# R-Sweke/DeepQ-Decoding

Hardware: AMD Instinct MI355X
Metric: env steps/sec + DQN updates/sec, d=5 depolarising, batch 4096, 1/2/4/8 GPU (higher is better)
Workload: dtype f32 (operands as 2 f16 pieces = 22 significant bits, 2 or 3 f16 MFMAs per product, f32 accumulate); 1 GPU; c3: d=5 DP p_phys=p_meas=0.011 depth=5, 4096 lattices/GPU, mode=loop; policy=eps-greedy over legal moves, eps=0.1, live Q-network, minibatch_per_gpu=4096, updates_per_vector_step=1, observations=patch words (d*d u32 per lattice), replay_ring_slots=257, network=conv 64x3s2-32x2-32x2, dense 512 (dropout .2), dueling, n_params=193283, grad_allreduce=none (1 GPU)

## Files before the change

deepq-decoding_amd/csrc/fused.hip:

```cpp
#include "qnet.h"
#include <type_traits>
#include <utility>

DQ_STAMP_READER(dq_dbg_read_fwd)

#ifndef CONV_PIN
#define CONV_PIN 1
#endif
#ifndef DENSE_PIN
#define DENSE_PIN 1
#endif
#ifndef CONV_APIPE
#define CONV_APIPE 1
#endif
#ifndef DENSE_XPIPE
#define DENSE_XPIPE 1
#endif
#ifndef CONV_SWZ
#define CONV_SWZ 0
#endif
#define A1_PS (CONV_SWZ ? 64 : 72)
#ifndef CONV1_PIPE
#define CONV1_PIPE 0
#endif
// ... 961 lines not shown
    const int NTQ = (A + 15) >> 4;
    float b3[KG3][4];
    f32x4 bias1[4];
#pragma unroll
    for (int ct = 0; ct < 4; ++ct)
        bias1[ct] = *reinterpret_cast<const f32x4u*>(J.params + a.b_off[0] + 64 * wave + 32 * (ct >> 1) + 8 * kq + 4 * (ct & 1));
    const int nt3 = NTQ > 0 ? NTQ : 1, parts = DENSE_WAVES / nt3, ct3 = wave % nt3, part = wave / nt3;
    const bool act3 = a.N3 > 0 && part < parts;
    const int col3 = 16 * ct3 + j;
    float bias3 = 0.f;
    auto load_b3 = [&]() {
        const float* w3q = reinterpret_cast<const float*>(J.packed + a.pk_w3q);
        bias3 = w3q[16 * KG3 * PW + col3];
#pragma unroll
        for (int g = 0; g < KG3; ++g)
#pragma unroll
            for (int s = 0; s < 4; ++s) b3[g][s] = w3q[(16 * g + 4 * kq + s) * PW + col3];
    };
    if (act3 && !LEAN) load_b3();
    const int rcol = tid & 63;
    float bias2r[(PW + 63) / 64];
#pragma unroll
    for (int cc = 0; cc < (PW + 63) / 64; ++cc) bias2r[cc] = J.params[a.b_off[1] + min(rcol + 64 * cc, a.N2 - 1)];
    __syncthreads();

    DQ_STAMP(DQ_TAG_DENSE_FWD, 3);
    auto hidden_pieces = [&](int u, F16x2 (&hb)[2]) {
        const int row = 16 * u + j;
        float rm = 0.f;
#pragma unroll
        for (int b = 0; b < 2; ++b) {
#pragma unroll
            for (int s = 0; s < 2; ++s) {
                const int ct = 2 * b + s;
                f32x4 v;
#pragma unroll
                for (int r = 0; r < 4; ++r) v[r] = fmaxf(f16x2_sum(acc[u][ct][0][r], acc[u][ct][1][r]) + bias1[ct][r], 0.f);
                if (J.keep_scale > 0.f) {
#pragma unroll
                    for (int r = 0; r < 4; ++r) v[r] = ((keepb[u] >> (8 * b + 4 * s + r)) & 1u) ? v[r] * J.keep_scale : 0.f;
                }
                range_max4(rm, v);
                u32 hp[2], lp[2];
                split_f16x2_pair(v[0], v[1], hp[0], lp[0]);
                split_f16x2_pair(v[2], v[3], hp[1], lp[1]);
                hb[b].h[2 * s] = hp[0]; hb[b].h[2 * s + 1] = hp[1];
                hb[b].l[2 * s] = lp[0]; hb[b].l[2 * s + 1] = lp[1];
            }
            if (J.h1_pl && row < ns && !DQ_EXP_NOSTORE) {
                unsigned short* gp = J.h1_pl + (size_t)(b0 + row) * DENSE_HID + 64 * wave + 32 * b + 8 * kq;
                *reinterpret_cast<u32x4*>(gp) = hb[b].h;
                *reinterpret_cast<u32x4*>(gp + (size_t)J.plane_rows * DENSE_HID) = hb[b].l;
            }
        }
        range_commit(rbad, rm);
    };
    if constexpr (LEAN) {
        static_assert(!LEAN || (ROWS / PR == 1 && UP == 2), "one reduction pass over both row tiles");
        F16x2 hbw[2][2];
        hidden_pieces(0, hbw[0]);
        hidden_pieces(1, hbw[1]);
#pragma unroll
        for (int uu = 0; uu < 2; ++uu) {
            f32x4 acc2[NT2][2];
#pragma unroll
            for (int t = 0; t < NT2; ++t) { acc2[t][0] = f32x4{0.f, 0.f, 0.f, 0.f}; acc2[t][1] = acc2[t][0]; }
#pragma unroll
            for (int b = 0; b < 2; ++b) {
                F16x2 wb[NT2];
#pragma unroll
                for (int t = 0; t < NT2; ++t) { wb[t].h = pk2[(b * NT2 + t) * PK_BLOCK]; wb[t].l = pk2[(b * NT2 + t) * PK_BLOCK + PK_LO]; }
#pragma unroll
                for (int t = 0; t < NT2; ++t) mma_f16x3(wb[t], hbw[uu][b], acc2[t][0], acc2[t][1]);
            }
#pragma unroll
            for (int t = 0; t < NT2; ++t)
                *reinterpret_cast<f32x4*>(s_part + (wave * PR + 16 * uu + j) * PWP + 16 * t + 4 * kq) = f16x2_sum(acc2[t][0], acc2[t][1]);
        }
    }
    if constexpr (WIDE2) {
        static_assert(!WIDE2 || (ROWS / PR == 1 && UP == 2), "one reduction pass over both row tiles");
        F16x2 hbw[2][2];
        F16x2 w2b[2][NTW];
        load_w2(w2, 0);
        load_w2(w2b, NTW);
        hidden_pieces(0, hbw[0]);
        hidden_pieces(1, hbw[1]);
#pragma unroll
        for (int hlf = 0; hlf < 2; ++hlf)
#pragma unroll
            for (int uu = 0; uu < 2; ++uu) {
                f32x4 acc2[NTW][2];
#pragma unroll
                for (int t = 0; t < NTW; ++t) { acc2[t][0] = f32x4{0.f, 0.f, 0.f, 0.f}; acc2[t][1] = acc2[t][0]; }
#pragma unroll
                for (int b = 0; b < 2; ++b)
#pragma unroll
                    for (int t = 0; t < NTW; ++t) mma_f16x3(hlf ? w2b[b][t] : w2[b][t], hbw[uu][b], acc2[t][0], acc2[t][1]);
#pragma unroll
                for (int t = 0; t < NTW; ++t)
                    *reinterpret_cast<f32x4*>(s_part + (wave * PR + 16 * uu + j) * PWP + 16 * (NTW * hlf + t) + 4 * kq) = f16x2_sum(acc2[t][0], acc2[t][1]);
            }
    }
#pragma unroll
    for (int pass = 0; pass < ROWS / PR; ++pass) {
#pragma unroll
        for (int uu = 0; uu < (WIDE2 || LEAN ? 0 : UP); ++uu) {
            const int u = pass * UP + uu, row = 16 * u + j;
            F16x2 hb[2];
            float rm = 0.f;
#pragma unroll
            for (int b = 0; b < 2; ++b) {
#pragma unroll
                for (int s = 0; s < 2; ++s) {
                    const int ct = 2 * b + s;
                    f32x4 v;
#pragma unroll
                    for (int r = 0; r < 4; ++r) v[r] = fmaxf(f16x2_sum(acc[u][ct][0][r], acc[u][ct][1][r]) + bias1[ct][r], 0.f);
                    if (J.keep_scale > 0.f) {
#pragma unroll
                        for (int r = 0; r < 4; ++r) v[r] = ((keepb[u] >> (8 * b + 4 * s + r)) & 1u) ? v[r] * J.keep_scale : 0.f;
                    }
                    range_max4(rm, v);
                    u32 hp[2], lp[2];
                    split_f16x2_pair(v[0], v[1], hp[0], lp[0]);
                    split_f16x2_pair(v[2], v[3], hp[1], lp[1]);
                    hb[b].h[2 * s] = hp[0]; hb[b].h[2 * s + 1] = hp[1];
                    hb[b].l[2 * s] = lp[0]; hb[b].l[2 * s + 1] = lp[1];
                }
                if (J.h1_pl && row < ns && !DQ_EXP_NOSTORE) {
                    unsigned short* gp = J.h1_pl + (size_t)(b0 + row) * DENSE_HID + 64 * wave + 32 * b + 8 * kq;
                    *reinterpret_cast<u32x4*>(gp) = hb[b].h;
                    *reinterpret_cast<u32x4*>(gp + (size_t)J.plane_rows * DENSE_HID) = hb[b].l;
                }
            }
            range_commit(rbad, rm);
            f32x4 acc2[NTW][2];
#pragma unroll
            for (int t = 0; t < NTW; ++t) { acc2[t][0] = f32x4{0.f, 0.f, 0.f, 0.f}; acc2[t][1] = acc2[t][0]; }
#pragma unroll
            for (int b = 0; b < 2; ++b)
#pragma unroll
                for (int t = 0; t < NTW; ++t) mma_f16x3(w2[b][t], hb[b], acc2[t][0], acc2[t][1]);
#pragma unroll
            for (int t = 0; t < NTW; ++t)
                *reinterpret_cast<f32x4*>(s_part + (wave * PR + 16 * uu + j) * PWP + 16 * t + 4 * kq) = f16x2_sum(acc2[t][0], acc2[t][1]);
        }
        if (pass == 0) { DQ_STAMP(DQ_TAG_DENSE_FWD, 4); }
        __syncthreads();
#pragma unroll
        for (int cc = 0; cc < (PW + 63) / 64; ++cc) {
            const int col = rcol + 64 * cc;
            if (col >= a.N2) continue;
#pragma unroll
            for (int rr = tid >> 6; rr < PR; rr += DENSE_THREADS / 64) {
                const int row = pass * PR + rr;
                float v = bias2r[cc];
#pragma unroll
                for (int w = 0; w < DENSE_WAVES; ++w) v += s_part[(w * PR + rr) * PWP + col];
                s_y2[row * a.ld2 + col] = v;
            }
        }
        __syncthreads();
        if (pass == 0) { DQ_STAMP(DQ_TAG_DENSE_FWD, 5); }
    }

    if (J.y2_pl) {
        const int per_row = J.small_ld >> 3, prs = J.small_ld == 64 ? 3 : 4;
        for (int i = tid; i < ROWS * per_row; i += DENSE_THREADS) {
            const int row = i >> prs, c8 = (i - (row << prs)) * 8;
            if (row >= ns) continue;
            const float* yp = s_y2 + row * a.ld2 + c8;
            const F16x2 o = split_f16x2(f32x4{yp[0], yp[1], yp[2], yp[3]}, f32x4{yp[4], yp[5], yp[6], yp[7]});
            unsigned short* gp = J.y2_pl + (size_t)(b0 + row) * J.small_ld + c8;
            *reinterpret_cast<u32x4*>(gp) = o.h;
            *reinterpret_cast<u32x4*>(gp + (size_t)J.plane_rows * J.small_ld) = o.l;
        }
    }
    DQ_STAMP(DQ_TAG_DENSE_FWD, 6);
    if (a.N3 > 0) {
        if (act3) {
            if constexpr (LEAN) load_b3();
            for (int u = part; u < RT; u += parts) {
                f32x4 acc3[2] = {{0.f, 0.f, 0.f, 0.f}, {0.f, 0.f, 0.f, 0.f}};
                const float* yrow = s_y2 + (16 * u + j) * a.ld2 + 4 * kq;
#pragma unroll
                for (int g = 0; g < KG3; ++g) {
                    const f32x4 av = *reinterpret_cast<const f32x4*>(yrow + 16 * g);
#pragma unroll
                    for (int s = 0; s < 4; ++s) acc3[s & 1] = MFMA16(av[s], b3[g][s], acc3[s & 1]);
                }
#pragma unroll
                for (int r = 0; r < 4; ++r) {
                    const int row = 16 * u + 4 * kq + r;
                    const float qv = (acc3[0][r] + acc3[1][r]) + bias3;
                    const bool live = col3 < A && row < ns;
                    if (live) J.q_out[(size_t)(b0 + row) * A + col3] = qv;
                    range_track_finite(rbad, live ? qv : 0.f);
                }
            }
        }
        DQ_STAMP(DQ_TAG_DENSE_FWD, 7);
    } else {
        DQ_STAMP(DQ_TAG_DENSE_FWD, 7);
        constexpr int RW = ROWS / DENSE_WAVES;
#pragma unroll
        for (int u = 0; u < RW; ++u) {
            const int row = wave + DENSE_WAVES * u;
            if (row >= ns) continue;
#pragma unroll
            for (int h = 0; h < 2; ++h) {
                const int c = lane + 64 * h;
                if (c < A) J.q_out[(size_t)(b0 + row) * A + c] = s_y2[row * a.ld2 + c];
            }
        }
    }
    range_report(rbad, a.range_flag);
    DQ_STAMP(DQ_TAG_DENSE_FWD, 8);
    DQ_STAMP_WG(DQ_TAG_DENSE_FWD, 1);
    DQ_STAMP_PAIR(3);
}

struct PackArgs {
    const float* params;
    u32x4* pk;
    int w1_off, K1, w2_off, w3_off, d1_off, d1_blocks;
    int d2_off, N2, NT2, KB2, d2_blocks, d2t_blocks, d1t_blocks, d1k;
    int perm_hw, perm_c;
    int pack_wgs, wide_blocks;
    int w3q_off, w3q_rows;
    int w3d_off, b3d_off, N3, n_actions;
    int wc_off, wc_waves;
    const int* ptab;
    int c1c_off, b1p_off, b1p_rows;
    int p_depth, p_C, b1_off;
    int c1w_off, c1w_blocks, p_kd;
    int c2w_off, c2w_blocks;
    int cdw_off, cdw_blocks;
    unsigned* range_flag;
    int n_params;
};

#define WCW_U 4
__device__ __forceinline__ void pack_wide_wc_block(const PackArgs& a, int block, float* s_w3) {
    const float* __restrict__ params = a.params;
    const int A = a.n_actions, N2 = a.N2, N3 = a.N3, lane = threadIdx.x & 63, wave = __builtin_amdgcn_readfirstlane((int)threadIdx.x >> 6);
    float* s_part = s_w3 + N2 * N3;
    const int n1_0 = min(block * WCW_U, DENSE_HID - WCW_U);
    float w2v[WCW_U][2];
#pragma unroll
    for (int q = 0; q < WCW_U; ++q)
#pragma unroll
        for (int h = 0; h < 2; ++h) {
            const float v = params[a.d2_off + (size_t)(n1_0 + q) * N2 + min(lane + 64 * h, N2 - 1)];
            w2v[q][h] = lane + 64 * h < N2 ? v : 0.f;
        }
    for (int base = 0; base < N2 * N3; base += 16 * 256) {
        float v[16];
#pragma unroll
        for (int u = 0; u < 16; ++u) v[u] = params[a.w3d_off + min(base + u * 256 + (int)threadIdx.x, N2 * N3 - 1)];
#pragma unroll
        for (int u = 0; u < 16; ++u) {
            const int i = base + u * 256 + (int)threadIdx.x;
            if (i < N2 * N3) s_w3[i] = v[u];
        }
    }
    __syncthreads();
    const int c0 = min(lane, N3 - 1), c1 = min(lane + 64, N3 - 1);
    float acc[WCW_U][2];
#pragma unroll
    for (int q = 0; q < WCW_U; ++q) acc[q][0] = acc[q][1] = 0.f;
    const int quarter = (N2 + 3) >> 2, r0 = wave * quarter, r1 = min(N2, r0 + quarter);
    for (int n2 = r0; n2 < r1; ++n2) {
        const float x0 = s_w3[n2 * N3 + c0], x1 = s_w3[n2 * N3 + c1];
#pragma unroll
        for (int q = 0; q < WCW_U; ++q) {
            const float w = __builtin_bit_cast(float, __builtin_amdgcn_readlane(__builtin_bit_cast(int, n2 < 64 ? w2v[q][0] : w2v[q][1]), n2 & 63));
            acc[q][0] = fmaf(w, x0, acc[q][0]);
            acc[q][1] = fmaf(w, x1, acc[q][1]);
        }
    }
#pragma unroll
    for (int q = 0; q < WCW_U; ++q) {
        s_part[(wave * WCW_U + q) * 128 + lane] = acc[q][0];
        s_part[(wave * WCW_U + q) * 128 + 64 + lane] = acc[q][1];
    }
    __syncthreads();
    if (block * WCW_U + wave >= DENSE_HID) return;
    const int n1 = block * WCW_U + wave;
    float P[2];
#pragma unroll
    for (int h = 0; h < 2; ++h)
        P[h] = ((s_part[(0 * WCW_U + wave) * 128 + 64 * h + lane] + s_part[(1 * WCW_U + wave) * 128 + 64 * h + lane]) +
                s_part[(2 * WCW_U + wave) * 128 + 64 * h + lane]) + s_part[(3 * WCW_U + wave) * 128 + 64 * h + lane];
    const bool in0 = lane >= 1 && lane <= A, in1 = lane + 64 <= A;
    float adv = (in0 ? P[0] : 0.f) + (in1 ? P[1] : 0.f);
    for (int m = 32; m >= 1; m >>= 1) adv += __shfl_xor(adv, m);
    const float v0 = __builtin_bit_cast(float, __builtin_amdgcn_readfirstlane(__builtin_bit_cast(int, P[0])));
    float* wc = reinterpret_cast<float*>(a.pk + a.wc_off);
    if (in0) wc[(size_t)(lane - 1) * DENSE_HID + n1] = (v0 + P[0]) - adv / (float)A;
    if (in1) wc[(size_t)(lane + 63) * DENSE_HID + n1] = (v0 + P[1]) - adv / (float)A;
}

__global__ __launch_bounds__(256) void pack_weights_kernel(PackArgs a) {
    extern __shared__ __attribute__((aligned(16))) float pack_smem[];
    if ((int)blockIdx.x < a.wide_blocks) { pack_wide_wc_block(a, (int)blockIdx.x, pack_smem); return; }
    const int pblock = (int)blockIdx.x - a.wide_blocks;
    const float* __restrict__ params = a.params;
    if (a.range_flag) {
        bool bad = false;
        for (int i = pblock * 256 + (int)threadIdx.x; i < a.n_params; i += a.pack_wgs * 256) bad = bad || !(fabsf(params[i]) < 65504.f);
        if (bad) atomicOr(a.range_flag, 2u);
    }
    u32x4* __restrict__ pk = a.pk;
    const int w2_off = a.w2_off, w3_off = a.w3_off, d1_off = a.d1_off, d1_blocks = a.d1_blocks;
    const int lane = threadIdx.x & 63, blk_id = pblock * 4 + (threadIdx.x >> 6), j = lane & 15, kb = lane >> 4;
    const int e_d1 = PK_TOTAL_BLOCKS + d1_blocks, e_d2 = e_d1 + a.d2_blocks, e_d2t = e_d2 + a.d2t_blocks, e_d1t = e_d2t + a.d1t_blocks;
    if (blk_id >= e_d1t) {
        const int r = blk_id - e_d1t;
        const int n_w3 = (a.w3q_rows ? a.w3q_rows + 1 : 0) + a.wc_waves;
        if (r >= n_w3) {
            const int rc = r - n_w3;
            if (!a.ptab) return;
            if (rc < 4) {
                float v[8];
#pragma unroll
                for (int e = 0; e < 8; ++e) {
                    const int row = a.ptab[PT_KROW + 8 * kb + e];
                    v[e] = row >= 0 ? params[a.w1_off + (size_t)row * 64 + 4 * j + rc] : 0.f;
                }
                const F16x2 o = split_f16x2(f32x4{v[0], v[1], v[2], v[3]}, f32x4{v[4], v[5], v[6], v[7]});
                u32x4* dst = pk + a.c1c_off + (size_t)rc * PK_BLOCK + lane;
                dst[0] = o.h; dst[PK_LO] = o.l;
            } else if (rc - 4 < a.b1p_rows) {
                const int pix = rc - 4, mask = a.ptab[PT_CONST + pix];
                double acc = (double)params[a.b1_off + lane];
                float w[5][8];
#pragma unroll
                for (int c = 0; c < 5; ++c) {
                    const int pos = a.ptab[PT_CPOS + c];
#pragma unroll
                    for (int pl = 0; pl < 8; ++pl) w[c][pl] = params[a.w1_off + (size_t)(pos * a.p_C + min(pl, a.p_depth - 1)) * 64 + lane];
                }
#pragma unroll
                for (int c = 0; c < 5; ++c) {
                    if (!((mask >> c) & 1)) continue;
#pragma unroll
                    for (int pl = 0; pl < 8; ++pl) if (pl < a.p_depth) acc += (double)w[c][pl];
                }
                reinterpret_cast<float*>(pk + a.b1p_off)[(size_t)pix * 64 + lane] = (float)acc;
            } else if (rc - 4 - a.b1p_rows < a.c1w_blocks) {
                const int bq = rc - 4 - a.b1p_rows, col = 16 * bq + j;
                float v[8], wc[8][8];
                int krow[8], cpos[8];
#pragma unroll
                for (int e = 0; e < 8; ++e) {
                    const int k = 8 * kb + e;
                    krow[e] = a.ptab[PT_KROW + k];
                    cpos[e] = a.ptab[PT_CPOS + min(max(k - a.p_kd, 0), 4)];
                }
#pragma unroll
                for (int e = 0; e < 8; ++e) {
                    const int k = 8 * kb + e;
                    const bool cst = k >= a.p_kd && k < a.p_kd + 5;
                    v[e] = k < a.p_kd ? params[a.w1_off + (size_t)max(krow[e], 0) * 64 + col] : k == a.p_kd + 5 ? params[a.b1_off + col] : 0.f;
#pragma unroll
                    for (int pl = 0; pl < 8; ++pl) wc[e][pl] = params[a.w1_off + (size_t)((cst ? cpos[e] : 0) * a.p_C + min(pl, a.p_depth - 1)) * 64 + col];
                }
#pragma unroll
                for (int e = 0; e < 8; ++e) {
                    const int k = 8 * kb + e;
                    if (k >= a.p_kd && k < a.p_kd + 5) {
                        double acc = 0.0;
#pragma unroll
                        for (int pl = 0; pl < 8; ++pl) if (pl < a.p_depth) acc += (double)wc[e][pl];
                        v[e] = (float)acc;
                    }
                }
                const F16x2 o = split_f16x2(f32x4{v[0], v[1], v[2], v[3]}, f32x4{v[4], v[5], v[6], v[7]});
                u32x4* dst = pk + a.c1w_off + (size_t)bq * PK_BLOCK + lane;
                dst[0] = o.h; dst[PK_LO] = o.l;
                if (a.range_flag) {
                    float pos = 0.f;
#pragma unroll
                    for (int e = 0; e < 8; ++e) pos += fmaxf(v[e], 0.f);
                    pos += __shfl_xor(pos, 16); pos += __shfl_xor(pos, 32);
                    if (!(pos < 65504.f)) atomicOr(a.range_flag, 2u);
                }
            } else if (rc - 4 - a.b1p_rows - a.c1w_blocks < a.c2w_blocks) {
                const int b = rc - 4 - a.b1p_rows - a.c1w_blocks, t = b & 1, ky = (b >> 1) & 1, qt = b >> 2;
                const float* w = params + w2_off + (size_t)((2 * ky + (kb >> 1)) * 64 + 16 * qt + 8 * (kb & 1)) * 32 + 2 * j + t;
                float v[8];
#pragma unroll
                for (int e = 0; e < 8; ++e) v[e] = w[(size_t)e * 32];
                const F16x2 o = split_f16x2(f32x4{v[0], v[1], v[2], v[3]}, f32x4{v[4], v[5], v[6], v[7]});
                u32x4* dst = pk + a.c2w_off + (size_t)b * PK_BLOCK + lane;
                dst[0] = o.h; dst[PK_LO] = o.l;
            } else if (rc - 4 - a.b1p_rows - a.c1w_blocks - a.c2w_blocks < a.cdw_blocks) {
                const int b = rc - 4 - a.b1p_rows - a.c1w_blocks - a.c2w_blocks;
                const bool c3 = b < 8;
                const int bb = c3 ? b : b - 8, tap = c3 ? bb >> 1 : bb >> 2, t = c3 ? bb & 1 : bb & 3, cin = c3 ? 32 : 64;
                const float* w = params + (c3 ? w3_off : w2_off) + (size_t)(tap * cin + 16 * t + j) * 32 + 8 * kb;
                float v[8];
#pragma unroll
                for (int e = 0; e < 8; ++e) v[e] = w[e];
                const F16x2 o = split_f16x2(f32x4{v[0], v[1], v[2], v[3]}, f32x4{v[4], v[5], v[6], v[7]});
                u32x4* dst = pk + a.cdw_off + (size_t)b * PK_BLOCK + lane;
                dst[0] = o.h; dst[PK_LO] = o.l;
            }
            return;
        }
        if (a.w3q_rows == 0) return;
        if (r > a.w3q_rows) {
            const int n1 = r - a.w3q_rows - 1;
            if (n1 >= a.wc_waves) return;
            const int A = a.n_actions, N2 = a.N2, N3 = a.N3;
            const __attribute__((address_space(4))) float* w2 = (const __attribute__((address_space(4))) float*)(uintptr_t)(params + a.d2_off + (size_t)n1 * N2);
            const float* W3 = params + a.w3d_off;
            const int c = min(lane, N3 - 1);
            float acc = 0.f, wv[64];
#pragma unroll
            for (int n2 = 0; n2 < 64; ++n2) wv[n2] = W3[(size_t)min(n2, N2 - 1) * N3 + c];
#pragma unroll
            for (int n2 = 0; n2 < 64; ++n2) acc = fmaf(n2 < N2 ? w2[n2] : 0.f, wv[n2], acc);
            float adv = (lane >= 1 && lane <= A) ? acc : 0.f;
            for (int m = 32; m >= 1; m >>= 1) adv += __shfl_xor(adv, m);
            const float v0 = __builtin_bit_cast(float, __builtin_amdgcn_readfirstlane(__builtin_bit_cast(int, acc)));
            if (lane >= 1 && lane <= A) reinterpret_cast<float*>(pk + a.wc_off)[(size_t)(lane - 1) * DENSE_HID + n1] = (v0 + acc) - adv / (float)A;
            return;
        }
        const int pw = 16 * a.NT2, A = a.n_actions;
        const bool live = r == a.w3q_rows || r < a.N2;
        const float* src = r == a.w3q_rows ? params + a.b3d_off : params + a.w3d_off + (size_t)min(r, a.N2 - 1) * a.N3;
        float va[2], sum = 0.f;
#pragma unroll
        for (int h = 0; h < 2; ++h) {
            const int c = lane + 64 * h;
            va[h] = (live && c < A) ? src[1 + c] : 0.f;
            sum += va[h];
        }
        for (int m = 32; m >= 1; m >>= 1) sum += __shfl_xor(sum, m);
        const float v0 = live ? src[0] : 0.f, mean = sum / (float)A;
        float* dst = reinterpret_cast<float*>(pk + a.w3q_off) + (size_t)r * pw;
        float* dstT = reinterpret_cast<float*>(pk + a.w3q_off) + (size_t)(a.w3q_rows + 1) * pw;
#pragma unroll
        for (int h = 0; h < 2; ++h) {
            const int c = lane + 64 * h;
            const float o = (live && c < A) ? (v0 + va[h]) - mean : 0.f;
            if (c < pw) { dst[c] = o; if (r < a.w3q_rows) dstT[(size_t)c * a.w3q_rows + r] = o; }
        }
        return;
    }
    float v[8];
    if (blk_id >= e_d2t) {
        const int tiles = a.d1k >> 4, b = blk_id - e_d2t, blk = b / tiles, ct = b - blk * tiles;
        int k = 16 * ct + j;
        if (a.perm_hw > 0) { const int pp = k / a.perm_c, c = k - pp * a.perm_c; k = c * a.perm_hw + pp; }
        const float* w = params + d1_off + (size_t)k * DENSE_HID + 32 * blk + 8 * kb;
#pragma unroll
        for (int e = 0; e < 8; ++e) v[e] = w[e];
    } else if (blk_id >= e_d2) {
        const int b = blk_id - e_d2, blk = b >> 5, ct = b & 31, n1 = 64 * (ct >> 2) + 4 * j + (ct & 3);
#pragma unroll
        for (int e = 0; e < 8; ++e) {
            const int n2 = 32 * blk + 8 * kb + e;
            v[e] = n2 < a.N2 ? params[a.d2_off + (size_t)n1 * a.N2 + n2] : 0.f;
        }
    } else if (blk_id >= e_d1) {
        const int b = blk_id - e_d1, blk = b / a.NT2, t = b - blk * a.NT2, col = 16 * t + j;
#pragma unroll
        for (int e = 0; e < 8; ++e) v[e] = col < a.N2 ? params[a.d2_off + (size_t)(32 * blk + 8 * kb + e) * a.N2 + col] : 0.f;
    } else if (blk_id >= PK_TOTAL_BLOCKS) {
        const int b = blk_id - PK_TOTAL_BLOCKS, kblk = b >> 5, ct = b & 31;
        const float* w = params + d1_off + 64 * (ct >> 2) + 32 * ((ct >> 1) & 1) + 8 * (j >> 2) + 4 * (ct & 1) + (j & 3);
#pragma unroll
        for (int e = 0; e < 8; ++e) {
            int k = 32 * kblk + 8 * kb + e;
            if (a.perm_hw > 0) { const int pp = k / a.perm_c, c = k - pp * a.perm_c; k = c * a.perm_hw + pp; }
            v[e] = w[(size_t)k * DENSE_HID];
        }
    } else if (blk_id < 16 + 8) {
        const bool c2 = blk_id < 16;
        const int b = c2 ? blk_id : blk_id - 16, blk = b >> 1, t = b & 1;
        const float* w = params + (c2 ? w2_off : w3_off);
#pragma unroll
        for (int e = 0; e < 8; ++e) v[e] = w[(size_t)(32 * blk + 8 * kb + e) * 32 + 2 * j + t];
    } else if (blk_id >= 48) {
        const int b = blk_id - 48, h = b >> 2, t = b & 3;
#pragma unroll
        for (int e = 0; e < 8; ++e) {
            const int k = 32 * h + 8 * kb + e;
            v[e] = k < a.K1 ? params[a.w1_off + (size_t)k * 64 + 4 * j + t] : 0.f;
        }
    } else {
        const bool c3 = blk_id < 32;
        const int b = c3 ? blk_id - 24 : blk_id - 32;
        const int t = b & 1, tap = (b >> 1) & 3, half = b >> 3, cin = c3 ? 32 : 64;
        const float* w = params + (c3 ? w3_off : w2_off) + (size_t)(tap * cin + 32 * half + 2 * j + t) * 32 + 8 * kb;
#pragma unroll
        for (int e = 0; e < 8; ++e) v[e] = w[e];
    }
    const F16x2 o = split_f16x2(f32x4{v[0], v[1], v[2], v[3]}, f32x4{v[4], v[5], v[6], v[7]});
    u32x4* dst = pk + (size_t)blk_id * PK_BLOCK + lane;
    dst[0] = o.h; dst[PK_LO] = o.l;
}

PackLayout fused_pack_layout(const dq_qnet* Q) {
    const int nc = Q->cfg.n_conv;
    const Layer &D1 = Q->L[nc], &D2 = Q->L[nc + 1];
    PackLayout P;
    P.NT2 = D2.nout <= 64 ? 4 : 8;
    P.KB2 = D2.nout <= 64 ? 2 : 4;
    P.d1_blocks = (D1.nin >> 5) * 32; P.d2_blocks = 16 * P.NT2; P.d2t_blocks = P.KB2 * 32; P.d1t_blocks = 16 * (D1.nin >> 4);
    P.dense1 = PK_TOTAL_U32X4;
    P.dense2 = P.dense1 + (size_t)P.d1_blocks * PK_BLOCK;
    P.dense2t = P.dense2 + (size_t)P.d2_blocks * PK_BLOCK;
    P.dense1t = P.dense2t + (size_t)P.d2t_blocks * PK_BLOCK;
    P.w3q = P.dense1t + (size_t)P.d1t_blocks * PK_BLOCK;
    P.w3q_rows = Q->cfg.dueling ? (D2.nout <= 64 ? 64 : 128) : 0;
    P.wc = P.w3q + ((size_t)(2 * P.w3q_rows + 1) * 16 * P.NT2 + 3) / 4;
    P.wc_rows = Q->cfg.dueling && (P.NT2 == 4 || (size_t)D2.nout * Q->L[nc + 2].nout * 4 <= 52 * 1024) ? Q->cfg.n_actions : 0;
    P.c1c = P.wc + (size_t)P.wc_rows * DENSE_HID / 4;
    P.b1p_rows = Q->L[0].rows <= 64 ? Q->L[0].rows : 0;
    P.b1p = P.c1c + (P.b1p_rows ? 4 * PK_BLOCK : 0);
    P.c1w = P.b1p + (size_t)P.b1p_rows * 64 / 4;
    P.c1w_blocks = P.b1p_rows ? 4 : 0;
    P.c2w = P.c1w + (size_t)P.c1w_blocks * PK_BLOCK;
    P.c2w_blocks = P.c1w_blocks ? 16 : 0;
    P.cdw = P.c2w + (size_t)P.c2w_blocks * PK_BLOCK;
    P.cdw_blocks = P.c1w_blocks ? 24 : 0;
    P.total = P.cdw + (size_t)P.cdw_blocks * PK_BLOCK;
    return P;
}
size_t fused_packed_w1t_u32x4(const dq_qnet* Q) { return fused_pack_layout(Q).total; }
size_t fused_packed_w2t_u32x4(const dq_qnet* Q) {
    const Layer& D1 = Q->L[Q->cfg.n_conv];
    return fused_packed_w1t_u32x4(Q) + ((size_t)D1.K * D1.N + 3) / 4;
}
size_t fused_packed_u32x4(const dq_qnet* Q) {
    const Layer& D2 = Q->L[Q->cfg.n_conv + 1];
    return fused_packed_w2t_u32x4(Q) + ((size_t)D2.K * D2.N + 3) / 4;
}

dq_status fused_pack_weights(const dq_qnet* Q, const float* params_dev, void* packed_dev, hipStream_t st) {
    DQ_REQUIRE(Q && params_dev && packed_dev, DQ_ERR_INVALID, "dq_qnet_pack: null argument");
    DQ_REQUIRE(fused_forward_supported(Q), DQ_ERR_UNSUPPORTED, "dq_qnet_pack: the fused chains do not cover this configuration");
    const int nc = Q->cfg.n_conv;
    const Layer &D1 = Q->L[nc], &D2 = Q->L[nc + 1];
    PackArgs a;
    memset(&a, 0, sizeof(a));
    a.params = params_dev; a.pk = static_cast<u32x4*>(packed_dev);
    a.w1_off = (int)Q->L[0].w_off; a.K1 = Q->L[0].K; a.w2_off = (int)Q->L[1].w_off; a.w3_off = (int)Q->L[2].w_off; a.d1_off = (int)D1.w_off; a.d1_blocks = (D1.nin >> 5) * 32;
    a.perm_hw = Q->flat_hw; a.perm_c = Q->flat_c;
    const PackLayout PL = fused_pack_layout(Q);
    a.d2_off = (int)D2.w_off; a.N2 = D2.nout; a.NT2 = PL.NT2; a.KB2 = PL.KB2; a.d2_blocks = PL.d2_blocks; a.d2t_blocks = PL.d2t_blocks;
    a.d1t_blocks = PL.d1t_blocks; a.d1k = D1.nin;
    a.w3q_off = (int)PL.w3q; a.w3q_rows = PL.w3q_rows; a.n_actions = Q->cfg.n_actions;
    if (Q->cfg.dueling) { const Layer& D3 = Q->L[nc + 2]; a.w3d_off = (int)D3.w_off; a.b3d_off = (int)D3.b_off; a.N3 = D3.nout; }
    a.wc_off = (int)PL.wc; a.wc_waves = PL.wc_rows && PL.NT2 == 4 ? DENSE_HID : 0;
    a.ptab = Q->patch_depth && PL.b1p_rows ? Q->ptab : nullptr;
    a.c1c_off = (int)PL.c1c; a.b1p_off = (int)PL.b1p; a.b1p_rows = PL.b1p_rows; a.p_depth = Q->patch_depth; a.p_C = Q->L[0].cin; a.b1_off = (int)Q->L[0].b_off;
    a.c1w_off = (int)PL.c1w; a.p_kd = Q->patch_kd; a.c1w_blocks = a.ptab && Q->patch_kd + 6 <= 32 ? PL.c1w_blocks : 0;
    a.c2w_off = (int)PL.c2w; a.c2w_blocks = a.c1w_blocks ? PL.c2w_blocks : 0;
    a.cdw_off = (int)PL.cdw; a.cdw_blocks = a.c1w_blocks ? PL.cdw_blocks : 0;
    a.pack_wgs = (PK_TOTAL_BLOCKS + PL.d1_blocks + PL.d2_blocks + PL.d2t_blocks + PL.d1t_blocks + (PL.w3q_rows ? PL.w3q_rows + 1 : 0) + a.wc_waves +
                  (a.ptab ? 4 + PL.b1p_rows + a.c1w_blocks + a.c2w_blocks + a.cdw_blocks : 0) + 3) / 4;
    const bool wide_wc = PL.wc_rows && PL.NT2 == 8;
    const int wide_blocks = wide_wc ? (DENSE_HID + WCW_U - 1) / WCW_U : 0;
    a.wide_blocks = wide_blocks;
    a.range_flag = fused_range_flag(Q); a.n_params = (int)Q->n_params;
    pack_weights_kernel<<<a.pack_wgs + wide_blocks, 256, wide_wc ? (size_t)a.N2 * a.N3 * 4 + 4 * WCW_U * 128 * 4 : 0, st>>>(a);
    DQ_LAUNCH_CHECK();
    return DQ_OK;
}

struct ConvPlan { int S, slot, off_mis, off_t1, off_a1, off_a2, off_fx, off_lut, KG1; size_t lds; };

static bool plan_conv(const dq_qnet* Q, ConvPlan* P, bool patch = false) {
    if (Q->cfg.n_conv != 3) return false;
    const Layer &L1 = Q->L[0], &L2 = Q->L[1], &L3 = Q->L[2];
    if (L1.cout != 64 || L1.K > 96) return false;
    if (L2.cin != 64 || L2.cout != 32 || L2.k != 2 || L2.s != 1) return false;
    if (L3.cin != 32 || L3.cout != 32 || L3.k != 2 || L3.s != 1) return false;
    if (patch && !Q->patch_depth) return false;
    P->KG1 = (L1.K + 15) / 16;
    if (P->KG1 < 3) P->KG1 = 3;
    const int in_bytes = Q->cfg.in_c * Q->cfg.in_h * Q->cfg.in_w;
    if (in_bytes >= (1 << 17)) return false;
    P->slot = patch ? 4 * Q->patch_stride : (in_bytes + 15 + 15 + 15) & ~15;
    const int a1ps = patch ? 64 : A1_PS;
    for (int pass = 0; pass < 2; ++pass) {
        const size_t budget = pass == 0 ? CONV_LDS_2PER_CU : CONV_LDS_MAX;
        for (int S = 8; S >= 1; S >>= 1) {
            size_t off = up16((size_t)S * P->slot);
            const size_t mis = off; off += up16((size_t)S * 4);
            const size_t t1 = off; off += up16((size_t)(S * L1.rows + (patch ? 16 : 0)) * 4);
            const size_t a2_bytes = up16((size_t)2 * S * L2.rows * 40 * 2);
            if (off < a2_bytes) off = a2_bytes;
            const size_t a1 = off; off += up16((size_t)2 * S * L1.rows * a1ps * 2);
            const size_t fx = off; off += CONV_SWZ ? up16((size_t)S * L1.rows + 16) : 0;
            const size_t lut = off; off += patch ? 4096 : 0;
            if (off <= budget && S * L1.rows <= CONV_ROWTAB) {
                P->S = S; P->off_mis = (int)mis; P->off_t1 = (int)t1; P->off_a1 = (int)a1; P->off_a2 = 0; P->off_fx = (int)fx; P->off_lut = (int)lut; P->lds = off;
                return true;
            }
        }
    }
    return false;
}

struct ConvPlanP { int S, slot, off_t1, off_obs1, off_a2b, off_a1, off_mis, off_lut, per_cu; size_t lds; };
static bool plan_conv_persist(const dq_qnet* Q, ConvPlanP* P, bool patch = false) {
    ConvPlan base;
    if (!plan_conv(Q, &base, patch)) return false;
    const Layer &L1 = Q->L[0], &L2 = Q->L[1];
    for (int pass = 0; pass < 2; ++pass) {
        const size_t budget = pass == 0 ? CONV_LDS_2PER_CU : CONV_LDS_MAX;
        for (int S = 8; S >= 1; S >>= 1) {
            const size_t obs = up16((size_t)S * base.slot), t1b = up16((size_t)(S * L1.rows + (patch ? 16 : 0)) * 4), a2b = up16((size_t)2 * S * L2.rows * 40 * 2);
            size_t core = a2b > obs ? a2b - obs : 0;
            if (core < t1b) core = t1b;
            size_t off = 2 * obs + core;
            const size_t a1 = off; off += up16((size_t)2 * (CONV1_PIPE ? (S * L1.rows + 15) & ~15 : S * L1.rows) * 64 * 2);
            const size_t mis = off; off += 2 * 16 * 4;
            const size_t t1c = off; off += t1b;
            const size_t lut = off; off += patch ? 4096 : 0;
            if (off <= budget && S * L1.rows <= CONV_ROWTAB) {
                P->S = S; P->slot = base.slot; P->off_t1 = (int)t1c; P->off_obs1 = (int)(obs + core); P->off_a2b = (int)(2 * obs + core - a2b);
                P->off_a1 = (int)a1; P->off_mis = (int)mis; P->off_lut = (int)lut; P->lds = off; P->per_cu = pass == 0 ? 2 : 1;
                return true;
            }
        }
    }
    return false;
}

bool fused_conv_row_tables(const dq_qnet* Q, int* tab) {
    ConvPlan P;
    if (!plan_conv(Q, &P)) return false;
    const Layer &L1 = Q->L[0], &L2 = Q->L[1], &L3 = Q->L[2];
    memset(tab, 0, sizeof(int) * CONV_FWD_TABS * CONV_ROWTAB);
    auto rows_of = [](const Layer& L) { return 8 * L.rows < CONV_ROWTAB ? 8 * L.rows : CONV_ROWTAB; };
    for (int m = 0; m < rows_of(L2); ++m) {
        const int s = m / L2.rows, pix = m % L2.rows, oy = pix / L2.ow, ox = pix % L2.ow;
        tab[3 * CONV_ROWTAB + m] = ((s * L2.ih + oy) * L2.iw + ox) * 64;
    }
    for (int m = 0; m < rows_of(L1); ++m) {
        const int s = m / L1.rows, pix = m % L1.rows, oy = pix / L1.ow, ox = pix % L1.ow;
        tab[m] = s << 20 | (CONV_SWZ ? (2 * (ox & 3)) << 17 : 0) | (oy * L1.s * L1.iw + ox * L1.s);
    }
    const Layer* Ls[2] = {&L2, &L3};
    for (int l = 0; l < 2; ++l)
        for (int m = 0; m < rows_of(*Ls[l]); ++m) {
            const int s = m / Ls[l]->rows, pix = m % Ls[l]->rows, oy = pix / Ls[l]->ow, ox = pix % Ls[l]->ow;
            tab[(1 + l) * CONV_ROWTAB + m] = l == 0 ? ((s * L2.ih + oy) * L2.iw + ox) * A1_PS | (CONV_SWZ ? (ox & 3) << 24 : 0)
                                                    : ((s * L3.ih + oy) * L3.iw + ox) * (L3.cin + 8);
        }
    return true;
}

bool fused_patch_supported(const dq_qnet* Q, int depth) {
    ConvPlan P;
    const Layer& L1 = Q->L[0];
    if (!plan_conv(Q, &P)) return false;
    if (L1.k != 3 || L1.s != 2 || L1.ih != L1.iw || !(L1.ih & 1) || L1.oh * L1.ow > 64) return false;
    if (depth < 1 || depth >= L1.cin) return false;
    return 4 * depth + (L1.cin - depth) <= 32;
}
void fused_patch_tables(const dq_qnet* Q, int depth, int stride_words, int* tab) {
    const Layer& L1 = Q->L[0];
    const int C = L1.cin, layers = C - depth, d = L1.oh, n = L1.ih, kd = 4 * depth + layers;
    memset(tab, 0, sizeof(int) * PT_TOTAL);
    for (int k = 0; k < 32; ++k) tab[PT_KROW + k] = -1;
    for (int k = 0; k < 96; ++k) tab[PT_SRC + k] = -1;
    for (int j = 0; j < depth; ++j)
        for (int c = 0; c < 4; ++c) {
            const int row = ((2 * (c >> 1)) * 3 + 2 * (c & 1)) * C + j;
            tab[PT_KROW + 4 * j + c] = row; tab[PT_SRC + row] = 4 * j + c;
        }
    for (int l = 0; l < layers; ++l) {
        const int row = (1 * 3 + 1) * C + depth + l;
        tab[PT_KROW + 4 * depth + l] = row; tab[PT_SRC + row] = 4 * depth + l;
    }
    const int cpos[5] = {0 * 3 + 1, 2 * 3 + 1, 1 * 3 + 0, 1 * 3 + 2, 1 * 3 + 1};
    for (int c = 0; c < 5; ++c) {
        tab[PT_CPOS + c] = cpos[c];
        for (int j = 0; j < depth; ++j) tab[PT_SRC + cpos[c] * C + j] = kd + c;
    }
    auto decoration = [&](int x, int y) {
        int v = 0;
        if ((x == 0 || x == n - 1) && (y & 1)) v = 1;
        if ((y == 0 || y == n - 1) && (x & 1)) v = 1;
        if ((x & 1) && (y & 1) && ((x + y) % 4 == 0)) v = 1;
        return v;
    };
    for (int oy = 0; oy < d; ++oy)
        for (int ox = 0; ox < d; ++ox) {
            int mask = 0;
            for (int c = 0; c < 5; ++c) mask |= decoration(2 * oy + cpos[c] / 3, 2 * ox + cpos[c] % 3) << c;
            tab[PT_CONST + oy * d + ox] = mask;
        }
    const int r1 = L1.rows, rows = 8 * r1 < CONV_ROWTAB ? 8 * r1 : CONV_ROWTAB;
    for (int m = 0; m < rows; ++m) {
        const int s = m / r1, pix = m % r1;
        tab[PT_FWD + m] = s << 20 | 4 * pix;
        tab[PT_BWD + m] = (s * stride_words + pix) | tab[PT_CONST + pix] << 16;
    }
    conv_wave_lane_table(Q, kd, tab + PT_CONST, tab + PT_WAVE);
    conv_bwd16_tables(Q, kd, stride_words, tab + PT_CONST, tab + PT_SRC, tab + PT_C16);
}

struct DensePlan { int ldx, ld2, ld3, off_x, off_h, off_part, off_y2, off_y3, NT2; size_t lds; };

static bool plan_dense(const dq_qnet* Q, DensePlan* P, int rt = 1) {
    const int nc = Q->cfg.n_conv;
    if (Q->cfg.n_ff != 1) return false;
    const Layer &D1 = Q->L[nc], &D2 = Q->L[nc + 1];
    if (D1.nout != DENSE_HID || (D1.nin & 31) || (Q->flat_c & 3)) return false;
    const int N2 = D2.nout, N3 = Q->cfg.dueling ? Q->L[nc + 2].nout : 0;
    if (N2 > 128 || N3 > 128) return false;
    const int rows = 16 * rt;
    P->NT2 = N2 <= 64 ? 4 : 8;
    if (rt > 2 && P->NT2 != 4) return false;
    P->ldx = D1.nin + 4;
    P->ld2 = 16 * P->NT2 + 4;
    P->ld3 = 16 * ((N3 + 15) / 16) + 1;
    size_t off = 0;
    const size_t xb = up16((size_t)2 * rows * (D1.nin + 8) * 2), pb = up16((size_t)DENSE_WAVES * (rows < DENSE_PR ? rows : DENSE_PR) * (16 * P->NT2 + 4) * 4);
    P->off_x = P->off_part = (int)off; off += xb > pb ? xb : pb;
    P->off_h = (int)off;
    P->off_y2 = (int)off; off += up16((size_t)rows * P->ld2 * 4);
    P->off_y3 = (int)off;
    P->lds = off;
    return off <= CONV_LDS_MAX;
}

bool fused_forward_supported(const dq_qnet* Q) {
    ConvPlan cp;
    DensePlan dp;
    return plan_conv(Q, &cp) && plan_dense(Q, &dp);
}

typedef void (*conv_kernel_t)(ConvChainArgs);
typedef void (*dense_kernel_t)(DenseChainArgs);

dq_status fused_forward_multi(dq_qnet* Q, int n_jobs, const dq_qnet_job* jobs, hipStream_t st) {
    ConvPlan cp;
    DensePlan dp;
    DQ_REQUIRE(n_jobs >= 1 && n_jobs <= FWD_MAX_JOBS, DQ_ERR_INVALID, "fused_forward: 1..%d jobs per launch", FWD_MAX_JOBS);
    const bool patch = (jobs[0].reserved & 1u) != 0;
    for (int i = 1; i < n_jobs; ++i)
        DQ_REQUIRE(((jobs[i].reserved & 1u) != 0) == patch, DQ_ERR_INVALID, "dq_qnet_forward_multi: the jobs of one launch must all read uint8 images or all read patch words");
    DQ_REQUIRE(!patch || Q->patch_depth, DQ_ERR_STATE, "dq_qnet_forward_multi: patch-word input without dq_qnet_set_patch_input");
    DQ_REQUIRE(plan_conv(Q, &cp, patch) && plan_dense(Q, &dp), DQ_ERR_UNSUPPORTED, "fused_forward: configuration not covered");
    conv_kernel_t ck = patch ? conv_chain_kernel<0> : cp.KG1 == 3 ? conv_chain_kernel<3> : cp.KG1 == 4 ? conv_chain_kernel<4> : cp.KG1 == 5 ? conv_chain_kernel<5> : conv_chain_kernel<6>;
    ConvPlanP pp;
    const char* pe = getenv("DQ_CONV_PERSIST");
    const int persist_env = pe ? atoi(pe) : 1;
    const char* pg = getenv("DQ_CONV_PERSIST_GRID");
    const int persist_grid = persist_env == 2 && pg ? atoi(pg) : 0;
    const bool can_persist = persist_env != 0 && plan_conv_persist(Q, &pp, patch) && pp.S == cp.S;
    const conv_kernel_t pk = patch ? conv_chain_pkernel<0> : cp.KG1 == 3 ? conv_chain_pkernel<3> : cp.KG1 == 4 ? conv_chain_pkernel<4> : cp.KG1 == 5 ? conv_chain_pkernel<5> : conv_chain_pkernel<6>;
    static unsigned long long attr_devs = 0;
    const unsigned long long dev_bit = dq_device_bit();
    if (!(attr_devs & dev_bit)) {
        const conv_kernel_t cks[5] = {conv_chain_kernel<3>, conv_chain_kernel<4>, conv_chain_kernel<5>, conv_chain_kernel<6>, conv_chain_kernel<0>};
        for (int i = 0; i < 5; ++i)
            DQ_HIP(hipFuncSetAttribute(reinterpret_cast<const void*>(cks[i]), hipFuncAttributeMaxDynamicSharedMemorySize, CONV_LDS_MAX));
        const conv_kernel_t pks[5] = {conv_chain_pkernel<3>, conv_chain_pkernel<4>, conv_chain_pkernel<5>, conv_chain_pkernel<6>, conv_chain_pkernel<0>};
        for (int i = 0; i < 5; ++i)
            DQ_HIP(hipFuncSetAttribute(reinterpret_cast<const void*>(pks[i]), hipFuncAttributeMaxDynamicSharedMemorySize, CONV_LDS_MAX));
        const dense_kernel_t dks[6] = {dense_chain_kernel<4, 4, 1>, dense_chain_kernel<8, 8, 1>, dense_chain_kernel<4, 4, 2>, dense_chain_kernel<4, 4, 4>,
                                       dense_chain_kernel<8, 8, 2>, dense_chain_kernel<4, 4, 2, true>};
        for (int i = 0; i < 6; ++i)
            DQ_HIP(hipFuncSetAttribute(reinterpret_cast<const void*>(dks[i]), hipFuncAttributeMaxDynamicSharedMemorySize, CONV_LDS_MAX));
        attr_devs |= dev_bit;
    }
    const int nc = Q->cfg.n_conv;
    const Layer &L1 = Q->L[0], &L2 = Q->L[1], &L3 = Q->L[2];
    const Layer &D1 = Q->L[nc], &D2 = Q->L[nc + 1];
    ConvChainArgs ca;
    DenseChainArgs da;
    memset(&ca, 0, sizeof(ca));
    memset(&da, 0, sizeof(da));
    ca.n_jobs = da.n_jobs = n_jobs; ca.S = cp.S;
    ca.C = L1.cin; ca.H = L1.ih; ca.W = L1.iw; ca.k1 = L1.k; ca.st1 = L1.s; ca.K1 = L1.K;
    ca.oh1 = L1.oh; ca.ow1 = L1.ow; ca.oh2 = L2.oh; ca.ow2 = L2.ow; ca.oh3 = L3.oh; ca.ow3 = L3.ow;
    for (int l = 0; l < 3; ++l) { ca.w_off[l] = (int)Q->L[l].w_off; ca.b_off[l] = (int)Q->L[l].b_off; }
    ca.kofftab = Q->kofftab; ca.rowtab = Q->kofftab + 96; ca.rowtab0 = patch ? Q->ptab + PT_FWD : ca.rowtab;
    ca.slot = cp.slot; ca.off_mis = cp.off_mis; ca.off_t1 = cp.off_t1; ca.off_a1 = cp.off_a1; ca.off_a2 = cp.off_a2; ca.off_fx = cp.off_fx; ca.off_lut = cp.off_lut;
    const PackLayout PL = fused_pack_layout(Q);
    ca.pk_c1c = (int)PL.c1c; ca.pk_b1p = (int)PL.b1p;
    da.K1 = D1.nin; da.perm_hw = Q->flat_hw; da.perm_c = Q->flat_c; da.pk_dense1 = (int)PL.dense1; da.pk_dense2 = (int)PL.dense2; da.pk_w3q = (int)PL.w3q;
    da.N2 = D2.nout; da.N3 = Q->cfg.dueling ? Q->L[nc + 2].nout : 0; da.n_actions = Q->cfg.n_actions;
    for (int l = 0; l < Q->n_layers - nc; ++l) { da.w_off[l] = (int)Q->L[nc + l].w_off; da.b_off[l] = (int)Q->L[nc + l].b_off; }
    int tiles16 = 0;
    for (int i = 0; i < n_jobs; ++i) tiles16 += (jobs[i].batch + 15) / 16;
    int n_cu = 256;
    {
        static int cached_cus = 0;
        if (!cached_cus) {
            int dev = 0;
            hipDeviceProp_t prop;
            if (hipGetDevice(&dev) == hipSuccess && hipGetDeviceProperties(&prop, dev) == hipSuccess) cached_cus = prop.multiProcessorCount;
            if (cached_cus <= 0) cached_cus = 256;
        }
        n_cu = cached_cus;
// ... 114 lines not shown
```

Before: 31.71 million env_steps/s.

## Overlap pack-kernel range check loads with weight packing and inline lookup tables

Moves the per-parameter range check in the weight-pack kernel from a serial prologue into a guard object. It issues its first batch of loads right after each block's weight loads and finishes the check after packing, so the two memory latencies overlap. Lookup-table reads (ptab krow/cpos) become closed-form arithmetic. Conditional loads are made unconditional with clamped indices so they can be issued together. Block order is reversed per slot and the check loop is unrolled by four, which raises register pressure and adds some redundant clamped loads.

Result: no change. 32.08 million env_steps/s (median of 6 runs) (+1.2%).

```diff
diff --git a/deepq-decoding_amd/csrc/fused.hip b/deepq-decoding_amd/csrc/fused.hip
--- a/deepq-decoding_amd/csrc/fused.hip
+++ b/deepq-decoding_amd/csrc/fused.hip
@@ -1287,16 +1287,45 @@
     if (in1) wc[(size_t)(lane + 63) * DENSE_HID + n1] = (v0 + P[1]) - adv / (float)A;
 }
 
-__global__ __launch_bounds__(256) void pack_weights_kernel(PackArgs a) {
-    extern __shared__ __attribute__((aligned(16))) float pack_smem[];
-    if ((int)blockIdx.x < a.wide_blocks) { pack_wide_wc_block(a, (int)blockIdx.x, pack_smem); return; }
-    const int pblock = (int)blockIdx.x - a.wide_blocks;
+struct PackGuard {
+    float g[4];
+    int i0;
+    bool issued;
+    __device__ __forceinline__ void issue(const PackArgs& a) {
+        if (issued || !a.range_flag) return;
+        issued = true;
+        const int stride = a.pack_wgs * 256;
+        if (i0 >= a.n_params) return;
+#pragma unroll
+        for (int u = 0; u < 4; ++u) { const int i = i0 + u * stride; g[u] = a.params[i < a.n_params ? i : i0]; }
+    }
+    __device__ __forceinline__ void finish(const PackArgs& a) {
+        if (!a.range_flag) return;
+        issue(a);
+        const int stride = a.pack_wgs * 256;
+        if (i0 >= a.n_params) return;
+        bool bad = false;
+#pragma unroll
+        for (int u = 0; u < 4; ++u) bad = bad || !(fabsf(g[u]) < 65504.f);
+        for (int i = i0 + 4 * stride; i < a.n_params; i += 4 * stride) {
+            float h[4];
+#pragma unroll
+            for (int u = 0; u < 4; ++u) { const int iu = i + u * stride; h[u] = a.params[iu < a.n_params ? iu : i]; }
+#pragma unroll
+            for (int u = 0; u < 4; ++u) bad = bad || !(fabsf(h[u]) < 65504.f);
+        }
+        if (bad) atomicOr(a.range_flag, 2u);
+    }
+};
+
+__device__ __forceinline__ int pt_krow(int k, int depth, int C, int kd) {
+    const int j = k >> 2, c = k & 3;
+    return k < 4 * depth ? ((2 * (c >> 1)) * 3 + 2 * (c & 1)) * C + j : k < kd ? 4 * C + depth + (k - 4 * depth) : -1;
+}
+__device__ __forceinline__ int pt_cpos(int c) { return (0x45371 >> (4 * c)) & 15; }
+
+__device__ __forceinline__ void pack_block(const PackArgs& a, int pblock, PackGuard& G) {
     const float* __restrict__ params = a.params;
-    if (a.range_flag) {
-        bool bad = false;
-        for (int i = pblock * 256 + (int)threadIdx.x; i < a.n_params; i += a.pack_wgs * 256) bad = bad || !(fabsf(params[i]) < 65504.f);
-        if (bad) atomicOr(a.range_flag, 2u);
-    }
     u32x4* __restrict__ pk = a.pk;
     const int w2_off = a.w2_off, w3_off = a.w3_off, d1_off = a.d1_off, d1_blocks = a.d1_blocks;
     const int lane = threadIdx.x & 63, blk_id = pblock * 4 + (threadIdx.x >> 6), j = lane & 15, kb = lane >> 4;
@@ -1311,9 +1340,11 @@
                 float v[8];
 #pragma unroll
                 for (int e = 0; e < 8; ++e) {
-                    const int row = a.ptab[PT_KROW + 8 * kb + e];
-                    v[e] = row >= 0 ? params[a.w1_off + (size_t)row * 64 + 4 * j + rc] : 0.f;
-                }
+                    const int row = pt_krow(8 * kb + e, a.p_depth, a.p_C, a.p_kd);
+                    const float w = params[a.w1_off + (size_t)max(row, 0) * 64 + 4 * j + rc];
+                    v[e] = row >= 0 ? w : 0.f;
+                }
+                G.issue(a);
                 const F16x2 o = split_f16x2(f32x4{v[0], v[1], v[2], v[3]}, f32x4{v[4], v[5], v[6], v[7]});
                 u32x4* dst = pk + a.c1c_off + (size_t)rc * PK_BLOCK + lane;
                 dst[0] = o.h; dst[PK_LO] = o.l;
@@ -1323,10 +1354,11 @@
                 float w[5][8];
 #pragma unroll
                 for (int c = 0; c < 5; ++c) {
-                    const int pos = a.ptab[PT_CPOS + c];
+                    const int pos = pt_cpos(c);
 #pragma unroll
                     for (int pl = 0; pl < 8; ++pl) w[c][pl] = params[a.w1_off + (size_t)(pos * a.p_C + min(pl, a.p_depth - 1)) * 64 + lane];
                 }
+                G.issue(a);
 #pragma unroll
                 for (int c = 0; c < 5; ++c) {
                     if (!((mask >> c) & 1)) continue;
@@ -1341,17 +1373,20 @@
 #pragma unroll
                 for (int e = 0; e < 8; ++e) {
                     const int k = 8 * kb + e;
-                    krow[e] = a.ptab[PT_KROW + k];
-                    cpos[e] = a.ptab[PT_CPOS + min(max(k - a.p_kd, 0), 4)];
+                    krow[e] = pt_krow(k, a.p_depth, a.p_C, a.p_kd);
+                    cpos[e] = pt_cpos(min(max(k - a.p_kd, 0), 4));
                 }
 #pragma unroll
                 for (int e = 0; e < 8; ++e) {
                     const int k = 8 * kb + e;
                     const bool cst = k >= a.p_kd && k < a.p_kd + 5;
-                    v[e] = k < a.p_kd ? params[a.w1_off + (size_t)max(krow[e], 0) * 64 + col] : k == a.p_kd + 5 ? params[a.b1_off + col] : 0.f;
+                    const bool data = k < a.p_kd, bias = k == a.p_kd + 5;
+                    const float wk = params[data ? a.w1_off + (size_t)max(krow[e], 0) * 64 + col : (size_t)a.b1_off + col];
+                    v[e] = data || bias ? wk : 0.f;
 #pragma unroll
                     for (int pl = 0; pl < 8; ++pl) wc[e][pl] = params[a.w1_off + (size_t)((cst ? cpos[e] : 0) * a.p_C + min(pl, a.p_depth - 1)) * 64 + col];
                 }
+                G.issue(a);
 #pragma unroll
                 for (int e = 0; e < 8; ++e) {
                     const int k = 8 * kb + e;
@@ -1378,6 +1413,7 @@
                 float v[8];
 #pragma unroll
                 for (int e = 0; e < 8; ++e) v[e] = w[(size_t)e * 32];
+                G.issue(a);
                 const F16x2 o = split_f16x2(f32x4{v[0], v[1], v[2], v[3]}, f32x4{v[4], v[5], v[6], v[7]});
                 u32x4* dst = pk + a.c2w_off + (size_t)b * PK_BLOCK + lane;
                 dst[0] = o.h; dst[PK_LO] = o.l;
@@ -1389,6 +1425,7 @@
                 float v[8];
 #pragma unroll
                 for (int e = 0; e < 8; ++e) v[e] = w[e];
+                G.issue(a);
                 const F16x2 o = split_f16x2(f32x4{v[0], v[1], v[2], v[3]}, f32x4{v[4], v[5], v[6], v[7]});
                 u32x4* dst = pk + a.cdw_off + (size_t)b * PK_BLOCK + lane;
                 dst[0] = o.h; dst[PK_LO] = o.l;
@@ -1406,6 +1443,7 @@
             float acc = 0.f, wv[64];
 #pragma unroll
             for (int n2 = 0; n2 < 64; ++n2) wv[n2] = W3[(size_t)min(n2, N2 - 1) * N3 + c];
+            G.issue(a);
 #pragma unroll
             for (int n2 = 0; n2 < 64; ++n2) acc = fmaf(n2 < N2 ? w2[n2] : 0.f, wv[n2], acc);
             float adv = (lane >= 1 && lane <= A) ? acc : 0.f;
@@ -1418,14 +1456,16 @@
         const bool live = r == a.w3q_rows || r < a.N2;
         const float* src = r == a.w3q_rows ? params + a.b3d_off : params + a.w3d_off + (size_t)min(r, a.N2 - 1) * a.N3;
         float va[2], sum = 0.f;
+        const float v0 = live ? src[0] : 0.f;
 #pragma unroll
         for (int h = 0; h < 2; ++h) {
             const int c = lane + 64 * h;
             va[h] = (live && c < A) ? src[1 + c] : 0.f;
             sum += va[h];
         }
+        G.issue(a);
         for (int m = 32; m >= 1; m >>= 1) sum += __shfl_xor(sum, m);
-        const float v0 = live ? src[0] : 0.f, mean = sum / (float)A;
+        const float mean = sum / (float)A;
         float* dst = reinterpret_cast<float*>(pk + a.w3q_off) + (size_t)r * pw;
         float* dstT = reinterpret_cast<float*>(pk + a.w3q_off) + (size_t)(a.w3q_rows + 1) * pw;
 #pragma unroll
@@ -1437,6 +1477,7 @@
         return;
     }
     float v[8];
+    G.issue(a);
     if (blk_id >= e_d2t) {
         const int tiles = a.d1k >> 4, b = blk_id - e_d2t, blk = b / tiles, ct = b - blk * tiles;
         int k = 16 * ct + j;
@@ -1449,12 +1490,16 @@
 #pragma unroll
         for (int e = 0; e < 8; ++e) {
             const int n2 = 32 * blk + 8 * kb + e;
-            v[e] = n2 < a.N2 ? params[a.d2_off + (size_t)n1 * a.N2 + n2] : 0.f;
+            const float w = params[a.d2_off + (size_t)n1 * a.N2 + min(n2, a.N2 - 1)];
+            v[e] = n2 < a.N2 ? w : 0.f;
         }
     } else if (blk_id >= e_d1) {
         const int b = blk_id - e_d1, blk = b / a.NT2, t = b - blk * a.NT2, col = 16 * t + j;
 #pragma unroll
-        for (int e = 0; e < 8; ++e) v[e] = col < a.N2 ? params[a.d2_off + (size_t)(32 * blk + 8 * kb + e) * a.N2 + col] : 0.f;
+        for (int e = 0; e < 8; ++e) {
+            const float w = params[a.d2_off + (size_t)(32 * blk + 8 * kb + e) * a.N2 + min(col, a.N2 - 1)];
+            v[e] = col < a.N2 ? w : 0.f;
+        }
     } else if (blk_id >= PK_TOTAL_BLOCKS) {
         const int b = blk_id - PK_TOTAL_BLOCKS, kblk = b >> 5, ct = b & 31;
         const float* w = params + d1_off + 64 * (ct >> 2) + 32 * ((ct >> 1) & 1) + 8 * (j >> 2) + 4 * (ct & 1) + (j & 3);
@@ -1475,7 +1520,8 @@
 #pragma unroll
         for (int e = 0; e < 8; ++e) {
             const int k = 32 * h + 8 * kb + e;
-            v[e] = k < a.K1 ? params[a.w1_off + (size_t)k * 64 + 4 * j + t] : 0.f;
+            const float w = params[a.w1_off + (size_t)min(k, a.K1 - 1) * 64 + 4 * j + t];
+            v[e] = k < a.K1 ? w : 0.f;
         }
     } else {
         const bool c3 = blk_id < 32;
@@ -1488,6 +1534,18 @@
     const F16x2 o = split_f16x2(f32x4{v[0], v[1], v[2], v[3]}, f32x4{v[4], v[5], v[6], v[7]});
     u32x4* dst = pk + (size_t)blk_id * PK_BLOCK + lane;
     dst[0] = o.h; dst[PK_LO] = o.l;
+}
+
+__global__ __launch_bounds__(256) void pack_weights_kernel(PackArgs a) {
+    extern __shared__ __attribute__((aligned(16))) float pack_smem[];
+    if ((int)blockIdx.x < a.wide_blocks) { pack_wide_wc_block(a, (int)blockIdx.x, pack_smem); return; }
+    const int slot = (int)blockIdx.x - a.wide_blocks;
+    PackGuard G;
+    G.i0 = slot * 256 + (int)threadIdx.x; G.issued = false;
+#pragma unroll
+    for (int u = 0; u < 4; ++u) G.g[u] = 0.f;
+    pack_block(a, a.pack_wgs - 1 - slot, G);
+    G.finish(a);
 }
 
 PackLayout fused_pack_layout(const dq_qnet* Q) {
```
